# kkty/kmer-sets-compression

Measured on AMD Instinct MI355X. Metric: Mk-mers/s processed in kmerset-multiple-compress; bytes/k-mer after SPSS, higher is better.
Workload: dtype u32

## Files before the change

### kmer-sets-compression_amd/csrc/ksh_decode.hip

```cpp
#include "ksh_internal.h"
#include "ksh_kmer.h"

#include <algorithm>
#include <cstdlib>
#include <string>
#include <vector>

namespace ksh {

constexpr int kDecThreads = 1024;
constexpr int kMaxLdsBuckets = 16384;
constexpr int kSortLdsBytes = 63488;
constexpr int kMaxSubBits = 11;
constexpr int kSortThreads = 1024;

__global__ __launch_bounds__(256) void k_str_bases(const uint32_t* __restrict__ lens, int64_t n,
                                                    int k, int64_t* __restrict__ bases) {
  const int64_t i = int64_t(blockIdx.x) * blockDim.x + threadIdx.x;
  if (i < n) bases[i] = int64_t(lens[i]) + k;
}

__global__ __launch_bounds__(256) void k_mark_ends(const int64_t* __restrict__ str_start,
                                                    int64_t n_strings,
                                                    unsigned long long* __restrict__ end_bits) {
  const int64_t i = int64_t(blockIdx.x) * blockDim.x + threadIdx.x;
  if (i >= n_strings) return;
  const int64_t p = str_start[i + 1] - 1;
  atomicOr(&end_bits[p >> 6], 1ull << (p & 63));
}

__global__ __launch_bounds__(256) void k_sum_lens(const uint32_t* __restrict__ lens, int64_t n,
                                                   unsigned long long* __restrict__ out) {
  unsigned long long acc = 0;
  for (int64_t i = int64_t(blockIdx.x) * blockDim.x + threadIdx.x; i < n;
       i += int64_t(gridDim.x) * blockDim.x)
    acc += lens[i];
#pragma unroll
  for (int d = 32; d >= 1; d >>= 1) acc += __shfl_xor(acc, d, 64);
  if ((threadIdx.x & 63) == 0 && acc) atomicAdd(out, acc);
}

template <typename KeyT, bool kScatter>
__global__ __launch_bounds__(kDecThreads) void k_decode(
    const uint64_t* __restrict__ words, int64_t n_words, int64_t n_bases,
    const unsigned long long* __restrict__ end_bits, int64_t n_end_words, int k, int key_bits,
    int n_buckets, int canonical_flag, int64_t words_per_group, uint32_t* __restrict__ hist_matrix,
    const int64_t* __restrict__ offsets, KeyT* __restrict__ keys) {
  extern __shared__ uint32_t lds_hist[];
  uint32_t* my_row = hist_matrix + int64_t(blockIdx.x) * n_buckets;
  for (int b = threadIdx.x; b < n_buckets; b += kDecThreads) lds_hist[b] = kScatter ? my_row[b] : 0u;
  __syncthreads();

  const int64_t w_begin = int64_t(blockIdx.x) * words_per_group;
  const int64_t w_end = min(w_begin + words_per_group, n_words);
  const uint64_t mask = kmer_mask(k);
  const uint64_t key_mask = (uint64_t(1) << key_bits) - 1;
  const uint64_t no_end_mask = (uint64_t(1) << (k - 1)) - 1;

  for (int64_t w = w_begin + threadIdx.x; w < w_end; w += kDecThreads) {
    const uint64_t w0 = words[w];
    const uint64_t w1 = (w + 1 < n_words) ? words[w + 1] : 0;
    const int64_t p0 = w << 5;
    const int64_t ew = p0 >> 6;
    const int esh = int(p0 & 63);
    uint64_t eb = end_bits[ew] >> esh;
    if (esh && ew + 1 < n_end_words) eb |= end_bits[ew + 1] << (64 - esh);

    uint64_t fw = (k <= 32) ? (w0 >> (64 - 2 * k)) : 0;
    uint64_t rc = revcomp(fw, k);
#pragma unroll 4
    for (int j = 0; j < 32; j++) {
      const int64_t p = p0 + j;
      const bool valid = (p + k <= n_bases) && (((eb >> j) & no_end_mask) == 0);
      if (valid) {
        const uint64_t cn = (canonical_flag && rc < fw) ? rc : fw;
        const uint32_t bucket = uint32_t(cn >> key_bits);
        if (kScatter) {
          const uint32_t rel = atomicAdd(&lds_hist[bucket], 1u);
          keys[offsets[bucket] + rel] = KeyT(cn & key_mask);
        } else {
          atomicAdd(&lds_hist[bucket], 1u);
        }
      }
      const int q = j + k;
      const uint64_t nb = q < 32 ? (w0 >> (62 - 2 * q)) & 3 : (w1 >> (62 - 2 * (q - 32))) & 3;
      fw = ((fw << 2) & mask) | nb;
      rc = (rc >> 2) | ((3 - nb) << (2 * (k - 1)));
    }
  }
  if (!kScatter) {
    __syncthreads();
    for (int b = threadIdx.x; b < n_buckets; b += kDecThreads) my_row[b] = lds_hist[b];
  }
}

constexpr int kDecSgBits = 7;
constexpr int kDecL1Threads = 1024;
template <typename KeyT>
struct DecL1 {
  static constexpr int kPer = sizeof(KeyT) == 8 ? 4 : 8;
  static constexpr int kTile = kDecL1Threads * kPer;
};
constexpr int kDecL2Threads = 256;
constexpr int kDecL2Per = 8;
constexpr int kDecL2Tile = kDecL2Threads * kDecL2Per;

template <typename KeyT>
__global__ __launch_bounds__(kDecL1Threads) void k_decode_l1(
    const uint64_t* __restrict__ words, int64_t n_words, int64_t n_bases,
    const unsigned long long* __restrict__ end_bits, int64_t n_end_words, int k, int key_bits, int n_bucket_bits,
    int canonical_flag, int64_t words_per_group, const uint32_t* __restrict__ hist_matrix,
    const int64_t* __restrict__ offsets, KeyT* __restrict__ tmp_keys, uint16_t* __restrict__ tmp_b) {
  constexpr int kSg = 1 << kDecSgBits;
  constexpr int kDecL1Per = DecL1<KeyT>::kPer, kDecL1Tile = DecL1<KeyT>::kTile;
  constexpr int kParts = 32 / kDecL1Per;
  __shared__ KeyT s_key[kDecL1Tile];
  __shared__ uint16_t s_bkt[kDecL1Tile];
  __shared__ uint32_t s_cur[kSg], s_cnt[kSg], s_lbase[kSg + 1];
  const int tid = threadIdx.x;
  const int nb = 1 << n_bucket_bits, lo_bits = n_bucket_bits - kDecSgBits;
  const uint32_t* my_row = hist_matrix + int64_t(blockIdx.x) * nb;
  if (tid < kSg) {
    uint32_t at = uint32_t(offsets[int64_t(tid) << lo_bits]);
    for (int bi = 0; bi < (1 << lo_bits); bi++) at += my_row[(tid << lo_bits) + bi];
    s_cur[tid] = at;
    s_cnt[tid] = 0;
  }
  const int64_t w_begin = int64_t(blockIdx.x) * words_per_group;
  const int64_t w_end = min(w_begin + words_per_group, n_words);
  const uint64_t mask = kmer_mask(k);
  const uint64_t key_mask = (uint64_t(1) << key_bits) - 1;
  const uint64_t no_end_mask = (uint64_t(1) << (k - 1)) - 1;
  __syncthreads();
  for (int64_t w0i = w_begin; w0i < w_end; w0i += kDecL1Tile / 32) {
    const int64_t w = w0i + tid / kParts;
    const int j0 = (tid % kParts) * kDecL1Per;
    KeyT key[kDecL1Per];
    uint32_t bkt[kDecL1Per], rank[kDecL1Per];
#pragma unroll
    for (int j = 0; j < kDecL1Per; j++) bkt[j] = 0xFFFFFFFFu;
    if (w < w_end) {
      const uint64_t w0 = words[w];
      const uint64_t w1 = (w + 1 < n_words) ? words[w + 1] : 0;
      const int64_t p0 = w << 5;
      const int64_t ew = p0 >> 6;
      const int esh = int(p0 & 63);
      uint64_t eb = end_bits[ew] >> esh;
      if (esh && ew + 1 < n_end_words) eb |= end_bits[ew + 1] << (64 - esh);
      const int top = 2 * (j0 + k);
      uint64_t fw = (top <= 64 ? (w0 >> (64 - top)) : ((w0 << (top - 64)) | (w1 >> (128 - top)))) & mask;
      uint64_t rc = revcomp(fw, k);
#pragma unroll
      for (int j = 0; j < kDecL1Per; j++) {
        const int jj = j0 + j;
        const int64_t p = p0 + jj;
        const bool valid = (p + k <= n_bases) && (((eb >> jj) & no_end_mask) == 0);
        if (valid) {
          const uint64_t cn = (canonical_flag && rc < fw) ? rc : fw;
          bkt[j] = uint32_t(cn >> key_bits);
          key[j] = KeyT(cn & key_mask);
          rank[j] = atomicAdd(&s_cnt[bkt[j] >> lo_bits], 1u);
        }
        const int q = jj + k;
        const uint64_t nbase = q < 32 ? (w0 >> (62 - 2 * q)) & 3 : (w1 >> (62 - 2 * (q - 32))) & 3;
        fw = ((fw << 2) & mask) | nbase;
        rc = (rc >> 2) | ((3 - nbase) << (2 * (k - 1)));
      }
    }
    __syncthreads();
    if (tid < 64) {
      static_assert(kSg == 128, "two super-buckets per lane of one wave");
      const uint32_t c0 = s_cnt[2 * tid], c1 = s_cnt[2 * tid + 1];
      uint32_t inc = c0 + c1;
#pragma unroll
      for (int d = 1; d < 64; d <<= 1) {
        const uint32_t o = __shfl_up(inc, d, 64);
        if (tid >= d) inc += o;
      }
      s_lbase[2 * tid] = inc - c0 - c1;
      s_lbase[2 * tid + 1] = inc - c1;
      if (tid == 63) s_lbase[kSg] = inc;
    }
    __syncthreads();
#pragma unroll
    for (int j = 0; j < kDecL1Per; j++) {
      if (bkt[j] == 0xFFFFFFFFu) continue;
      const uint32_t pos = s_lbase[bkt[j] >> lo_bits] + rank[j];
      s_key[pos] = key[j];
      s_bkt[pos] = uint16_t(bkt[j]);
    }
    __syncthreads();
    const int tile_n = int(s_lbase[kSg]);
    for (int i = tid; i < tile_n; i += kDecL1Threads) {
      const uint32_t sg = uint32_t(s_bkt[i]) >> lo_bits;
      const uint32_t dst = s_cur[sg] + (uint32_t(i) - s_lbase[sg]);
      tmp_keys[dst] = s_key[i];
      tmp_b[dst] = s_bkt[i];
    }
    __syncthreads();
    if (tid < kSg) {
      s_cur[tid] += s_cnt[tid];
      s_cnt[tid] = 0;
    }
    __syncthreads();
  }
}

template <typename KeyT>
__global__ __launch_bounds__(kDecL2Threads) void k_decode_l2(int64_t n, int n_bucket_bits,
                                                             const int64_t* __restrict__ offsets,
                                                             const KeyT* __restrict__ tmp_keys,
                                                             const uint16_t* __restrict__ tmp_b,
                                                             uint32_t* __restrict__ cursor, KeyT* __restrict__ keys) {
  constexpr int kBins = 2 * kDecL2Threads;
  __shared__ KeyT s_key[kDecL2Tile];
  __shared__ uint16_t s_bin[kDecL2Tile];
  __shared__ uint32_t s_cnt[kBins], s_lbase[kBins], s_gbase[kBins];
  __shared__ uint32_t s_wave[kDecL2Threads / 64];
  __shared__ uint32_t s_first;
  const int tid = threadIdx.x;
  const int lo_bits = n_bucket_bits - kDecSgBits;
  const int64_t p0 = int64_t(blockIdx.x) * kDecL2Tile;
  const int tile_n = int(min<int64_t>(kDecL2Tile, n - p0));
  s_cnt[2 * tid] = 0;
  s_cnt[2 * tid + 1] = 0;
  if (tid == 0) s_first = (uint32_t(tmp_b[p0]) >> lo_bits) << lo_bits;
  __syncthreads();
  const uint32_t base_b = s_first;
  const uint32_t n_bins = min<uint32_t>(uint32_t(kBins), (2u << lo_bits));
  KeyT mine[kDecL2Per];
  uint32_t bin[kDecL2Per], rank[kDecL2Per];
#pragma unroll
  for (int j = 0; j < kDecL2Per; j++) {
    const int i = tid + j * kDecL2Threads;
    bin[j] = 0xFFFFFFFFu;
    if (i >= tile_n) continue;
    mine[j] = tmp_keys[p0 + i];
    const uint32_t b = tmp_b[p0 + i];
    if (b - base_b < n_bins) {
      bin[j] = b - base_b;
      rank[j] = atomicAdd(&s_cnt[bin[j]], 1u);
    } else {
      keys[uint32_t(offsets[b]) + atomicAdd(&cursor[b], 1u)] = mine[j];
    }
  }
  __syncthreads();
  {
    const uint32_t c0 = s_cnt[2 * tid], c1 = s_cnt[2 * tid + 1];
    uint32_t inc = c0 + c1;
    const int lane = tid & 63, wv = tid >> 6;
#pragma unroll
    for (int d = 1; d < 64; d <<= 1) {
      const uint32_t o = __shfl_up(inc, d, 64);
      if (lane >= d) inc += o;
    }
    if (lane == 63) s_wave[wv] = inc;
    __syncthreads();
    uint32_t before = inc - (c0 + c1);
    for (int w = 0; w < wv; w++) before += s_wave[w];
    s_lbase[2 * tid] = before;
    s_lbase[2 * tid + 1] = before + c0;
    s_gbase[2 * tid] = c0 ? uint32_t(offsets[base_b + 2 * tid]) + atomicAdd(&cursor[base_b + 2 * tid], c0) : 0u;
    s_gbase[2 * tid + 1] = c1 ? uint32_t(offsets[base_b + 2 * tid + 1]) + atomicAdd(&cursor[base_b + 2 * tid + 1], c1) : 0u;
  }
  __syncthreads();
#pragma unroll
  for (int j = 0; j < kDecL2Per; j++) {
    if (bin[j] == 0xFFFFFFFFu) continue;
    const uint32_t pos = s_lbase[bin[j]] + rank[j];
    s_key[pos] = mine[j];
    s_bin[pos] = uint16_t(bin[j]);
  }
  __syncthreads();
  const uint32_t staged = s_lbase[kBins - 1] + s_cnt[kBins - 1];
  for (uint32_t i = tid; i < staged; i += kDecL2Threads) {
    const uint32_t b = s_bin[i];
    keys[s_gbase[b] + (i - s_lbase[b])] = s_key[i];
  }
}

constexpr int kColTeams = 16;
__global__ __launch_bounds__(64 * kColTeams) void k_hist_columns(uint32_t* __restrict__ hist_matrix,
                                                                  int64_t n_groups, int n_buckets,
                                                                  int64_t* __restrict__ totals,
                                                                  unsigned long long* __restrict__ max_total) {
  __shared__ uint32_t team_total[kColTeams][64];
  const int lane = threadIdx.x & 63, team = threadIdx.x >> 6;
  const int b = blockIdx.x * 64 + lane;
  const int64_t per_team = (n_groups + kColTeams - 1) / kColTeams;
  const int64_t g0 = min(int64_t(team) * per_team, n_groups), g1 = min(g0 + per_team, n_groups);
  uint32_t run = 0;
  if (b < n_buckets)
    for (int64_t g = g0; g < g1; g++) run += hist_matrix[g * n_buckets + b];
  team_total[team][lane] = run;
  __syncthreads();
  if (b >= n_buckets) return;
  uint32_t before = 0, all = 0;
#pragma unroll
  for (int t2 = 0; t2 < kColTeams; t2++) {
    const uint32_t v = team_total[t2][lane];
    if (t2 < team) before += v;
    all += v;
  }
  run = before;
  for (int64_t g = g0; g < g1; g++) {
    uint32_t* cell = hist_matrix + g * n_buckets + b;
    const uint32_t c = *cell;
    *cell = run;
    run += c;
  }
  if (team == 0) {
    totals[b] = all;
    unsigned long long m = all;
    if (int(blockIdx.x + 1) * 64 <= n_buckets) {
#pragma unroll
      for (int d = 32; d >= 1; d >>= 1) {
        const unsigned long long o = __shfl_xor(m, d, 64);
        m = o > m ? o : m;
      }
      if (lane == 0 && max_total) atomicMax(max_total, m);
    } else if (max_total) {
      atomicMax(max_total, m);
    }
  }
}

struct SortLds {
  uint32_t sub_cnt[(1 << kMaxSubBits) + 1];
  int wave_cnt[kSortThreads / 64];
  int wave_below[kSortThreads / 64];
  int overflow;
  int kept;
};

template <typename KeyT>
__device__ void block_sort_into_lds(const KeyT* __restrict__ src, int cnt, int eff_bits,
                                    KeyT* __restrict__ lds, SortLds* __restrict__ sh) {
  int bits = 0;
  while ((4 << bits) < cnt && bits < kMaxSubBits) bits++;
  if (bits > eff_bits) bits = eff_bits;
  const int n_sub = 1 << bits;
  const int shift = eff_bits - bits;
  for (int i = threadIdx.x; i <= n_sub; i += kSortThreads) sh->sub_cnt[i] = 0;
  if (threadIdx.x == 0) sh->overflow = 0;
  constexpr int kSortRegs = 8;
  const bool in_regs = cnt <= kSortRegs * kSortThreads;
  KeyT held[kSortRegs];
  if (in_regs) {
#pragma unroll
    for (int u = 0; u < kSortRegs; u++) {
      const int i = int(threadIdx.x) + u * kSortThreads;
      if (i < cnt) held[u] = src[i];
    }
  }
  __syncthreads();
// ... 407 lines not shown
  int64_t* offw = wide ? st.coarse : d_offsets;

  const unsigned sb = unsigned((s->n_strings + 255) / 256);
  hipLaunchKernelGGL(k_str_bases, dim3(sb), dim3(256), 0, ctx->stream, s->d_lens, s->n_strings, g->k,
                     st.str_start);
  KSH_TRY(scan_exclusive_i64(ctx, st.str_start, st.str_start, s->n_strings,
                             st.str_start + s->n_strings));
  KSH_HIP(hipMemsetAsync(st.end_bits, 0, size_t(n_end_words) * 8, ctx->stream));
  hipLaunchKernelGGL(k_mark_ends, dim3(sb), dim3(256), 0, ctx->stream, st.str_start, s->n_strings,
                     st.end_bits);
  hipLaunchKernelGGL((k_decode<KeyT, false>), dim3(unsigned(groups)), dim3(kDecThreads),
                     size_t(nbw) * 4, ctx->stream, s->d_words, n_words, s->n_bases, st.end_bits,
                     n_end_words, g->k, kbw, int(nbw), canonical_flag, wpg, st.hist, nullptr,
                     static_cast<KeyT*>(nullptr));
  unsigned long long* d_max = reinterpret_cast<unsigned long long*>(st.totals + nbw + 1);
  KSH_HIP(hipMemsetAsync(d_max, 0, 8, ctx->stream));
  hipLaunchKernelGGL(k_hist_columns, dim3(unsigned((nbw + 63) / 64)), dim3(64 * kColTeams), 0, ctx->stream,
                     st.hist, groups, int(nbw), st.totals, d_max);
  KSH_TRY(scan_exclusive_i64(ctx, st.totals, offw, nbw, offw + nbw));
  if (wide)
    hipLaunchKernelGGL(k_broadcast_coarse, dim3(unsigned(nb / 256 + 1)), dim3(256), 0, ctx->stream, st.coarse,
                       g->n_bucket_bits - kCoarseBits, nb, d_offsets);
  KSH_HIP(hipGetLastError());
  KSH_HIP(hipMemcpyAsync(ctx->h_pinned, offw + nbw, 8, hipMemcpyDeviceToHost, ctx->stream));
  KSH_HIP(hipMemcpyAsync(ctx->h_pinned + 1, st.str_start + s->n_strings, 8, hipMemcpyDeviceToHost,
                         ctx->stream));
  KSH_HIP(hipMemcpyAsync(ctx->h_pinned + 2, d_max, 8, hipMemcpyDeviceToHost, ctx->stream));
  KSH_HIP(hipStreamSynchronize(ctx->stream));
  ctx->dec_max_bucket = ctx->h_pinned[2];
  if (ctx->h_pinned[1] != s->n_bases)
    return fail(KSH_INVALID_ARGUMENT, "spss: sum of string lengths (%lld) != n_bases (%lld)",
                (long long)ctx->h_pinned[1], (long long)s->n_bases);
  *n_keys = ctx->h_pinned[0];
  ctx->dec_words = n_words;
  ctx->dec_groups = groups;
  plan_done(*n_keys);
  return KSH_OK;
}

int decode_claim_plan(ksh_ctx* ctx, const char* who, const ksh_geom* g, const ksh_spss_view* s, int canonical_flag,
                      const int64_t* d_offsets) {
  if (!ctx->dec_valid)
    return fail(KSH_FAILED_PRECONDITION, "%s without a pending ksh_spss_decode_plan on this context (none made, "
                                         "replaced, failed, or already written)", who);
  const ksh_spss_view& v = ctx->dec_view;
  if (v.d_words != s->d_words || v.d_lens != s->d_lens || v.n_strings != s->n_strings || v.n_bases != s->n_bases)
    return fail(KSH_FAILED_PRECONDITION, "%s: the pending ksh_spss_decode_plan was made for another container", who);
  if (!same_geom(ctx->dec_geom, *g) || ctx->dec_canonical != (canonical_flag != 0))
    return fail(KSH_FAILED_PRECONDITION, "%s: the pending ksh_spss_decode_plan was made with another geometry "
                                         "(k, N, key bytes) or canonical flag", who);
  if (ctx->dec_offsets != d_offsets)
    return fail(KSH_FAILED_PRECONDITION, "%s: d_offsets is not the buffer the pending ksh_spss_decode_plan filled",
                who);
  return KSH_OK;
}

template <typename KeyT>
int scatter_sort(ksh_ctx* ctx, const ksh_spss_view* s, const DecodeState& st, int k, int nbits_w, int kbw,
                 int canonical_flag, const int64_t* offsets, KeyT* keys, int cutoff, bool want_below,
                 int64_t** new_off, int64_t** below) {
  const int64_t nb = int64_t(1) << nbits_w;
  int64_t n_words, n_end_words, groups, wpg;
  decode_geometry(s, &n_words, &n_end_words, &groups, &wpg);
  static const bool direct = [] {
    const char* e = getenv("KSH_DECODE_SCATTER");
    return e && std::string(e) == "direct";
  }();
  static const int64_t two_level_min = [] {
    const char* e = getenv("KSH_DECODE_L2_MIN");
    return e ? std::max<int64_t>(1024, atoll(e)) : int64_t(1) << 20;
  }();
  if (!direct && ctx->dec_kmers >= two_level_min && nbits_w > kDecSgBits && nbits_w <= 15 &&
      ctx->dec_kmers < int64_t(0xFFFFFFF0)) {
    void* tmp = nullptr;
    const size_t tk = (size_t(ctx->dec_kmers) * sizeof(KeyT) + 255) & ~size_t(255);
    KSH_TRY(pool_alloc(ctx, tk + size_t(ctx->dec_kmers) * 2 + size_t(nb) * 4 + 256, &tmp));
    KeyT* tmp_keys = static_cast<KeyT*>(tmp);
    uint16_t* tmp_b = reinterpret_cast<uint16_t*>(static_cast<char*>(tmp) + tk);
    uint32_t* cursor = reinterpret_cast<uint32_t*>(static_cast<char*>(tmp) + tk + ((size_t(ctx->dec_kmers) * 2 + 255) & ~size_t(255)));
    KSH_HIP(hipMemsetAsync(cursor, 0, size_t(nb) * 4, ctx->stream));
    hipLaunchKernelGGL((k_decode_l1<KeyT>), dim3(unsigned(groups)), dim3(kDecL1Threads), 0, ctx->stream, s->d_words,
                       n_words, s->n_bases, st.end_bits, n_end_words, k, kbw, nbits_w,
                       canonical_flag, wpg, st.hist, offsets, tmp_keys, tmp_b);
    hipLaunchKernelGGL((k_decode_l2<KeyT>), dim3(unsigned((ctx->dec_kmers + kDecL2Tile - 1) / kDecL2Tile)),
                       dim3(kDecL2Threads), 0, ctx->stream, ctx->dec_kmers, nbits_w, offsets, tmp_keys, tmp_b,
                       cursor, keys);
    pool_free(ctx, tmp);
  } else {
    hipLaunchKernelGGL((k_decode<KeyT, true>), dim3(unsigned(groups)), dim3(kDecThreads),
                       size_t(nb) * 4, ctx->stream, s->d_words, n_words, s->n_bases, st.end_bits,
                       n_end_words, k, kbw, int(nb), canonical_flag, wpg, st.hist, offsets,
                       keys);
  }
  KeyT* scratch = nullptr;
  {
    const int64_t max_bucket = ctx->dec_max_bucket;
    if (max_bucket > int64_t(kSortLdsBytes / sizeof(KeyT))) {
      void* ptr = nullptr;
      KSH_TRY(pool_alloc(ctx, size_t(ctx->dec_kmers) * sizeof(KeyT), &ptr));
      scratch = static_cast<KeyT*>(ptr);
    }
  }
  KSH_TRY(arena_layout(ctx, 1u << 16, [&](Carver& c) {
    *new_off = c.take<int64_t>(size_t(nb + 1));
    *below = c.take<int64_t>(size_t(nb + 1));
  }));
  {
    const uint32_t bit = lds_opt_in_bit<KeyT>(kLdsBucketSort);
    if (!(ctx->lds_opt_in & bit)) {
      KSH_HIP(hipFuncSetAttribute(reinterpret_cast<const void*>(k_bucket_sort<KeyT>),
                                  hipFuncAttributeMaxDynamicSharedMemorySize, kSortLdsBytes));
      ctx->lds_opt_in |= bit;
    }
  }
  hipLaunchKernelGGL((k_bucket_sort<KeyT>), dim3(unsigned(nb)), dim3(kSortThreads), kSortLdsBytes, ctx->stream,
                     offsets, keys, scratch, st.totals, kbw, cutoff, want_below ? *below : nullptr);
  if (scratch) pool_free(ctx, scratch);
  KSH_HIP(hipGetLastError());
  return KSH_OK;
}

template <typename KeyT, typename CT>
int decode_write_wide(ksh_ctx* ctx, const ksh_geom* g, const ksh_spss_view* s, int canonical_flag,
                      int64_t* d_offsets, void* d_keys, int64_t* n_keys, int cutoff, int64_t* n_below) {
  const int64_t nb = n_buckets(g), nbc = int64_t(1) << kCoarseBits;
  const int sub_bits = g->n_bucket_bits - kCoarseBits, cbits = 2 * g->k - kCoarseBits;
  int64_t n_words, n_end_words, groups, wpg;
  decode_geometry(s, &n_words, &n_end_words, &groups, &wpg);
  DecodeState st;
  KSH_TRY(decode_carve(ctx, DecodeShape{groups, nbc, n_end_words, s->n_strings, true}, &st));
  KeyT* keys = static_cast<KeyT*>(d_keys);
  constexpr bool in_place = sizeof(CT) == sizeof(KeyT);
  CT* comp = reinterpret_cast<CT*>(d_keys);
  if (!in_place) {
    void* ptr = nullptr;
    KSH_TRY(pool_alloc(ctx, size_t(ctx->dec_kmers) * sizeof(CT), &ptr));
    comp = static_cast<CT*>(ptr);
  }
  int64_t *new_off = nullptr, *below = nullptr;
  KSH_TRY(scatter_sort<CT>(ctx, s, st, g->k, kCoarseBits, cbits, canonical_flag, st.coarse, comp, cutoff,
                           n_below != nullptr, &new_off, &below));
  KSH_TRY(scan_exclusive_i64(ctx, st.totals, new_off, nbc, new_off + nbc));
  if (n_below) KSH_TRY(scan_exclusive_i64(ctx, below, below, nbc, below + nbc));
  hipLaunchKernelGGL((k_fine_offsets<CT>), dim3(unsigned(nb / 256 + 1)), dim3(256), 0, ctx->stream, st.coarse,
                     new_off, comp, sub_bits, key_bits(g), nb, d_offsets);
  KSH_HIP(hipMemcpyAsync(ctx->h_pinned, new_off + nbc, 8, hipMemcpyDeviceToHost, ctx->stream));
  if (n_below)
    KSH_HIP(hipMemcpyAsync(ctx->h_pinned + 1, below + nbc, 8, hipMemcpyDeviceToHost, ctx->stream));
  KSH_HIP(hipStreamSynchronize(ctx->stream));
  const int64_t kept = ctx->h_pinned[0];
  if (n_below) *n_below = ctx->h_pinned[1];
  const uint64_t key_mask = key_bits(g) >= 64 ? ~uint64_t(0) : (uint64_t(1) << key_bits(g)) - 1;
  void* tmp = nullptr;
  const CT* src = comp;
  if (in_place && kept != ctx->dec_kmers) {
    KSH_TRY(device_alloc(ctx, size_t(ctx->dec_kmers) * sizeof(CT), &tmp));
    KSH_HIP(hipMemcpyAsync(tmp, comp, size_t(ctx->dec_kmers) * sizeof(CT), hipMemcpyDeviceToDevice, ctx->stream));
    src = static_cast<const CT*>(tmp);
  }
  hipLaunchKernelGGL((k_narrow_buckets<CT, KeyT>), dim3(unsigned(nbc)), dim3(256), 0, ctx->stream, st.coarse,
                     new_off, src, keys, key_mask);
  KSH_HIP(hipGetLastError());
  if (!in_place) pool_free(ctx, comp);
  if (tmp) {
    KSH_HIP(hipStreamSynchronize(ctx->stream));
    KSH_HIP(hipFree(tmp));
  }
// ... 122 lines not shown
```

### kmer-sets-compression_amd/csrc/ksh_encode.hip

```cpp
#include "ksh_internal.h"
#include "ksh_dsu.h"
#include "ksh_kmer.h"

#include <algorithm>
#include <cstddef>
#include <cstdlib>
#include <string>
#ifdef KSH_EDGES_DEBUG
#include <cstdio>
#include <vector>
#endif

namespace ksh {

#ifndef KSH_RULER_SHIFT
#define KSH_RULER_SHIFT 5
#endif
constexpr int kRulerShift = KSH_RULER_SHIFT;
constexpr uint32_t kRulerEvery = 1u << kRulerShift;

constexpr uint32_t kNone = 0xFFFFFFFFu;
constexpr uint32_t kMulti = 0xFFFFFFFEu;

#ifndef KSH_JUMP_HOPS
// ... 202 lines not shown

constexpr int kColTeams = 16;
__global__ __launch_bounds__(64 * kColTeams) void k_rc_columns(uint32_t* __restrict__ hist_matrix, int64_t n_rows,
                                                                int nb, int64_t* __restrict__ totals) {
  __shared__ uint32_t team_total[kColTeams][64];
  const int lane = threadIdx.x & 63, team = threadIdx.x >> 6;
  const int b = blockIdx.x * 64 + lane;
  const int64_t per_team = (n_rows + kColTeams - 1) / kColTeams;
  const int64_t g0 = min(int64_t(team) * per_team, n_rows), g1 = min(g0 + per_team, n_rows);
  uint32_t run = 0;
  if (b < nb)
    for (int64_t g = g0; g < g1; g++) run += hist_matrix[g * nb + b];
  team_total[team][lane] = run;
  __syncthreads();
  if (b >= nb) return;
  uint32_t before = 0, all = 0;
#pragma unroll
  for (int t2 = 0; t2 < kColTeams; t2++) {
    const uint32_t v = team_total[t2][lane];
    if (t2 < team) before += v;
    all += v;
  }
  run = before;
  for (int64_t g = g0; g < g1; g++) {
    uint32_t* cell = hist_matrix + g * nb + b;
    const uint32_t c = *cell;
    *cell = run;
    run += c;
  }
  if (team == 0) totals[b] = all;
}

template <typename KeyT>
__global__ __launch_bounds__(1024) void k_rc_scatter(DevSet<KeyT> set, int nbits, int round_bits, int round,
                                                      int64_t per_row,
                                                      const uint32_t* __restrict__ hist_matrix,
                                                      const int64_t* __restrict__ goff,
                                                      RcRecord<KeyT>* __restrict__ rec) {
  extern __shared__ uint32_t lds_hist[];
  const int nb = 1 << nbits;
  const uint32_t* my_row = hist_matrix + int64_t(blockIdx.x) * nb;
  for (int b = threadIdx.x; b < nb; b += blockDim.x) lds_hist[b] = uint32_t(goff[b]) + my_row[b];
  const int64_t t_begin = int64_t(blockIdx.x) * per_row;
  const int64_t t_end = min(t_begin + per_row, set.n);
  __syncthreads();
  if (t_begin >= t_end) return;
  const int64_t b_first = set.bucket_of(t_begin), b_last = set.bucket_of(t_end - 1);
  const int k = set.k, low_bits = 2 * set.k - 2 - nbits;
  const uint64_t low_mask = (uint64_t(1) << low_bits) - 1;
  for (int64_t t = t_begin + threadIdx.x; t < t_end; t += blockDim.x) {
    const uint64_t key = uint64_t(set.keys[t]);
    const uint32_t grp = uint32_t(revcomp(key, k) >> low_bits) & uint32_t(nb - 1);
    if (int(grp >> (nbits - round_bits)) != round) continue;
    int64_t lo = b_first, hi = b_last;
    while (lo < hi) {
      const int64_t mid = (lo + hi + 1) >> 1;
      if (set.off[mid] <= t) lo = mid; else hi = mid - 1;
    }
    const uint64_t rx = revcomp((uint64_t(lo) << set.key_bits) | key, k);
    const uint32_t dst = atomicAdd(&lds_hist[grp], 1u);
    RcRecord<KeyT> r;
    r.key = KeyT(((rx >> (2 * k - 2)) << low_bits) | (rx & low_mask));
    r.t = uint32_t(t);
    rec[dst] = r;
  }
}

constexpr int kSgBits = 7;
constexpr int kL1Threads = 1024;
constexpr int kL2Threads = 256;
constexpr int kL2Per = 8;
constexpr int kL2Tile = kL2Threads * kL2Per;

template <typename KeyT, int kPer>
__global__ __launch_bounds__(kL1Threads) void k_rc_scatter_l1(DevSet<KeyT> set, int nbits, int64_t per_row,
                                                               const uint32_t* __restrict__ hist_matrix,
                                                               const int64_t* __restrict__ goff,
                                                               RcRecord<KeyT>* __restrict__ tmp_rec,
                                                               uint16_t* __restrict__ tmp_g) {
  constexpr int kTile = kL1Threads * kPer;
  constexpr int kSg = 1 << kSgBits;
  __shared__ RcRecord<KeyT> s_rec[kTile];
  __shared__ uint16_t s_g[kTile];
  __shared__ uint32_t s_cur[kSg], s_cnt[kSg], s_lbase[kSg + 1];
  constexpr int kOffCap = 1024;
  __shared__ int64_t s_off[kOffCap];
  const int tid = threadIdx.x;
  const int nb = 1 << nbits, lo_bits = nbits - kSgBits;
  const uint32_t* my_row = hist_matrix + int64_t(blockIdx.x) * nb;
  if (tid < kSg) {
    uint32_t at = uint32_t(goff[int64_t(tid) << lo_bits]);
    for (int gi = 0; gi < (1 << lo_bits); gi++) at += my_row[(tid << lo_bits) + gi];
    s_cur[tid] = at;
    s_cnt[tid] = 0;
  }
  const int64_t t_begin = int64_t(blockIdx.x) * per_row;
  const int64_t t_end = min(t_begin + per_row, set.n);
  __syncthreads();
  if (t_begin >= t_end) return;
  const int64_t b_first = set.bucket_of(t_begin), b_last = set.bucket_of(t_end - 1);
  const int k = set.k, low_bits = 2 * set.k - 2 - nbits;
  const uint64_t low_mask = (uint64_t(1) << low_bits) - 1;
  const int n_span = int(min<int64_t>(b_last - b_first + 1, kOffCap + 1));
  const bool off_staged = n_span <= kOffCap;
  if (off_staged)
    for (int j = tid; j < n_span; j += kL1Threads) s_off[j] = set.off[b_first + j];
  __syncthreads();
  for (int64_t t0 = t_begin; t0 < t_end; t0 += kTile) {
    const int tile_n = int(min<int64_t>(kTile, t_end - t0));
    RcRecord<KeyT> mine[kPer];
    uint32_t grp[kPer], rank[kPer];
#pragma unroll
    for (int j = 0; j < kPer; j++) {
      const int64_t t = t0 + tid + j * kL1Threads;
      grp[j] = 0xFFFFFFFFu;
      if (t >= t_end) continue;
      const uint64_t key = uint64_t(set.keys[t]);
      int64_t lo = b_first, hi = b_last;
      if (off_staged) {
        int l2 = 0, h2 = n_span - 1;
        while (l2 < h2) {
          const int mid = (l2 + h2 + 1) >> 1;
          if (s_off[mid] <= t) l2 = mid; else h2 = mid - 1;
        }
        lo = b_first + l2;
      } else {
        while (lo < hi) {
          const int64_t mid = (lo + hi + 1) >> 1;
          if (set.off[mid] <= t) lo = mid; else hi = mid - 1;
        }
      }
      const uint64_t rx = revcomp((uint64_t(lo) << set.key_bits) | key, k);
      grp[j] = uint32_t(rx >> low_bits) & uint32_t(nb - 1);
      mine[j].key = KeyT(((rx >> (2 * k - 2)) << low_bits) | (rx & low_mask));
      mine[j].t = uint32_t(t);
      rank[j] = atomicAdd(&s_cnt[grp[j] >> lo_bits], 1u);
    }
    __syncthreads();
    if (tid < 64) {
      static_assert(kSg == 128, "two super-groups per lane of one wave");
      const uint32_t c0 = s_cnt[2 * tid], c1 = s_cnt[2 * tid + 1];
      uint32_t inc = c0 + c1;
#pragma unroll
      for (int d = 1; d < 64; d <<= 1) {
        const uint32_t o = __shfl_up(inc, d, 64);
        if (tid >= d) inc += o;
      }
      s_lbase[2 * tid] = inc - c0 - c1;
      s_lbase[2 * tid + 1] = inc - c1;
    }
    __syncthreads();
#pragma unroll
    for (int j = 0; j < kPer; j++) {
      if (grp[j] == 0xFFFFFFFFu) continue;
      const uint32_t pos = s_lbase[grp[j] >> lo_bits] + rank[j];
      s_rec[pos] = mine[j];
      s_g[pos] = uint16_t(grp[j]);
    }
    __syncthreads();
    for (int i = tid; i < tile_n; i += kL1Threads) {
      const uint32_t sg = uint32_t(s_g[i]) >> lo_bits;
      const uint32_t dst = s_cur[sg] + (uint32_t(i) - s_lbase[sg]);
      tmp_rec[dst] = s_rec[i];
      tmp_g[dst] = s_g[i];
    }
    __syncthreads();
    if (tid < kSg) {
      s_cur[tid] += s_cnt[tid];
      s_cnt[tid] = 0;
    }
    __syncthreads();
  }
}

template <typename KeyT>
__global__ __launch_bounds__(kL2Threads) void k_rc_scatter_l2(int64_t n, int nbits, const int64_t* __restrict__ goff,
                                                               const RcRecord<KeyT>* __restrict__ tmp_rec,
                                                               const uint16_t* __restrict__ tmp_g,
                                                               uint32_t* __restrict__ cursor,
                                                               RcRecord<KeyT>* __restrict__ rec) {
  constexpr int kBins = 512;
  __shared__ RcRecord<KeyT> s_rec[kL2Tile];
  __shared__ uint16_t s_bin[kL2Tile];
  __shared__ uint32_t s_cnt[kBins], s_lbase[kBins], s_gbase[kBins];
  __shared__ uint32_t s_first;
  const int tid = threadIdx.x;
  const int lo_bits = nbits - kSgBits;
  const int64_t p0 = int64_t(blockIdx.x) * kL2Tile;
  const int tile_n = int(min<int64_t>(kL2Tile, n - p0));
  for (int b = tid; b < kBins; b += kL2Threads) s_cnt[b] = 0;
  if (tid == 0) s_first = (uint32_t(tmp_g[p0]) >> lo_bits) << lo_bits;
  __syncthreads();
  const uint32_t base_g = s_first;
  const uint32_t n_bins = min<uint32_t>(uint32_t(kBins), (2u << lo_bits));
  RcRecord<KeyT> mine[kL2Per];
  uint32_t bin[kL2Per], rank[kL2Per];
#pragma unroll
  for (int j = 0; j < kL2Per; j++) {
    const int i = tid + j * kL2Threads;
    bin[j] = 0xFFFFFFFFu;
    if (i >= tile_n) continue;
    mine[j] = tmp_rec[p0 + i];
    const uint32_t g = tmp_g[p0 + i];
    if (g - base_g < n_bins) {
      bin[j] = g - base_g;
      rank[j] = atomicAdd(&s_cnt[bin[j]], 1u);
    } else {
      rec[uint32_t(goff[g]) + atomicAdd(&cursor[g], 1u)] = mine[j];
    }
  }
  __syncthreads();
  {
    static_assert(kBins == 2 * kL2Threads, "two bins per thread");
    __shared__ uint32_t s_wave[kL2Threads / 64];
    const uint32_t c0 = s_cnt[2 * tid], c1 = s_cnt[2 * tid + 1];
    uint32_t inc = c0 + c1;
    const int lane = tid & 63, wv = tid >> 6;
#pragma unroll
    for (int d = 1; d < 64; d <<= 1) {
      const uint32_t o = __shfl_up(inc, d, 64);
      if (lane >= d) inc += o;
    }
    if (lane == 63) s_wave[wv] = inc;
    __syncthreads();
    uint32_t before = inc - (c0 + c1);
    for (int w = 0; w < wv; w++) before += s_wave[w];
    s_lbase[2 * tid] = before;
    s_lbase[2 * tid + 1] = before + c0;
    s_gbase[2 * tid] = c0 ? uint32_t(goff[base_g + 2 * tid]) + atomicAdd(&cursor[base_g + 2 * tid], c0) : 0u;
    s_gbase[2 * tid + 1] = c1 ? uint32_t(goff[base_g + 2 * tid + 1]) + atomicAdd(&cursor[base_g + 2 * tid + 1], c1) : 0u;
  }
  __syncthreads();
#pragma unroll
  for (int j = 0; j < kL2Per; j++) {
    if (bin[j] == 0xFFFFFFFFu) continue;
    const uint32_t pos = s_lbase[bin[j]] + rank[j];
    s_rec[pos] = mine[j];
    s_bin[pos] = uint16_t(bin[j]);
  }
  __syncthreads();
  uint32_t staged = 0;
  for (int b = 0; b < kBins; b++) staged += s_cnt[b];
  for (uint32_t i = tid; i < staged; i += kL2Threads) {
    const uint32_t b = s_bin[i];
    rec[s_gbase[b] + (i - s_lbase[b])] = s_rec[i];
  }
}

template <typename KeyT>
__device__ int64_t lower_bound_kmer(const DevSet<KeyT>& set, uint64_t value) {
  const int64_t b = int64_t(value >> set.key_bits);
  if (b >= set.n_buckets) return set.n;
  const KeyT key = KeyT(value & set.key_mask());
  int64_t lo, hi;
  set.probe_range(b, key, &lo, &hi);
  while (lo < hi) {
    const int64_t mid = (lo + hi) >> 1;
    if (set.keys[mid] < key) lo = mid + 1; else hi = mid;
  }
  return lo;
}

__device__ __forceinline__ void mark_hit(uint32_t* slot, uint32_t v) {
  if (atomicCAS(slot, kNone, v) != kNone) *reinterpret_cast<volatile uint32_t*>(slot) = kMulti;
}

constexpr int kRcSegs = 16;

template <typename KeyT>
__global__ __launch_bounds__(256) void k_rc_bounds(DevSet<KeyT> set, int nbits, int64_t* __restrict__ pb,
                                                    int64_t* __restrict__ pb0) {
  const int64_t i = int64_t(blockIdx.x) * blockDim.x + threadIdx.x;
  const int64_t n_pb = int64_t(2 * kRcSegs) << nbits;
  if (i < n_pb) {
    const uint64_t grp = uint64_t(i) >> 5, seg = (uint64_t(i) >> 1) & 15, which = uint64_t(i) & 1;
    const uint64_t prefix = (seg << nbits) | grp;
    pb[i] = lower_bound_kmer(set, (prefix + which) << (2 * set.k - 4 - nbits));
  } else if (pb0 && i - n_pb < (int64_t(2) << nbits)) {
    const uint64_t j = uint64_t(i - n_pb);
    pb0[j] = lower_bound_kmer(set, ((j >> 1) + (j & 1)) << (2 * set.k - nbits));
  }
}
struct RcBatch {
  int64_t seg_lo[kRcSegs], seg_hi[kRcSegs];
  int64_t win_lo[kRcSegs];
  int win_len[kRcSegs];
  int win_off[kRcSegs];
  int idx_off[kRcSegs];
  int idx_shift[kRcSegs];
  unsigned long long packed[kRcSegs];
  int used;
  int next_seg;
  int64_t next_pos;
};

template <typename KeyT, int kRcThreads>
__global__ __launch_bounds__(kRcThreads, (kRcThreads >= 512 ? 8 : (kRcThreads >= 128 ? kRcThreads / 128 : 1))) void k_adj_rc(
    DevSet<KeyT> set, int gbits, const int64_t* __restrict__ goff, const RcRecord<KeyT>* __restrict__ rec,
    const int64_t* __restrict__ pb, const int64_t* __restrict__ pb0, int cap, uint32_t* __restrict__ rc0,
    uint32_t* __restrict__ rc1, int* __restrict__ batched, int pass1_cap, int* __restrict__ taken) {
  extern __shared__ __attribute__((aligned(16))) unsigned char lds_raw[];
  KeyT* skeys = reinterpret_cast<KeyT*>(lds_raw);
  uint32_t* slots = reinterpret_cast<uint32_t*>(lds_raw + size_t(cap) * sizeof(KeyT));
  uint16_t* sidx = reinterpret_cast<uint16_t*>(lds_raw + size_t(cap) * (sizeof(KeyT) + 4));
  __shared__ RcBatch bt;
  __shared__ int64_t prev_bounds[2 * kRcSegs];
  static_assert(kRcThreads % kRcSegs == 0, "pass 1 deals the ranges out to sixteen teams");
  constexpr int kTeam = kRcThreads / kRcSegs;
  const int tid = threadIdx.x, lane = tid % kTeam, wave = tid / kTeam;
  const int64_t grp = blockIdx.x;
  const int k = set.k, low_bits = 2 * set.k - 2 - gbits;
  const int extra = gbits - int(2 * set.k - set.key_bits);
  const uint64_t low_mask = (uint64_t(1) << low_bits) - 1;
  const uint64_t kmask = kmer_mask(k);
  const int64_t r0 = goff[grp], r1 = goff[grp + 1];
  if (r1 - r0 <= int64_t(pass1_cap)) return;
  if (pass1_cap >= 0 && threadIdx.x == 0) *taken = 1;
  const int64_t p0_lo = pb0 ? pb0[2 * grp] : set.off[grp], p0_hi = pb0 ? pb0[2 * grp + 1] : set.off[grp + 1];
  const uint64_t gkey_top = extra > 0 ? (uint64_t(grp) & ((uint64_t(1) << extra) - 1)) << (set.key_bits - extra) : 0;
  KSH_PMARK_WAVE(2);
  if (tid < 2 * kRcSegs) prev_bounds[tid] = pb[2 * kRcSegs * grp + tid];
  KSH_PMARK(1, 0);
  for (int pass = 0; pass < 2; pass++) {
    const int n_seg = pass == 0 ? 1 : kRcSegs;
    const int seg_bits = (pass == 0 ? set.key_bits : set.key_bits - 4) - extra;
// ... 3403 lines not shown
```

Measured before the change: 28600.

## Prefetch next tile inputs and overlap global atomics in decode/encode scatter kernels

The decode L1 kernel now loads the next tile's words and end-bit words into registers while the current tile is processed. The encode L1 kernel prefetches keys one tile ahead, tracks the bucket index incrementally instead of running a fresh binary search per element, and folds the cursor update into the scan so two barriers per tile go away. The L2 scatter kernels issue all global loads before the shared-memory barrier, start the global cursor atomics before the prefix scan, and the decode L2 tile doubles for 32-bit keys. The aim is to hide memory latency and cut barriers, at the cost of more registers and LDS, which may lower occupancy.

```diff
diff --git a/kmer-sets-compression_amd/csrc/ksh_decode.hip b/kmer-sets-compression_amd/csrc/ksh_decode.hip
--- a/kmer-sets-compression_amd/csrc/ksh_decode.hip
+++ b/kmer-sets-compression_amd/csrc/ksh_decode.hip
@@ -102,8 +102,11 @@
   static constexpr int kTile = kDecL1Threads * kPer;
 };
 constexpr int kDecL2Threads = 256;
-constexpr int kDecL2Per = 8;
-constexpr int kDecL2Tile = kDecL2Threads * kDecL2Per;
+template <typename KeyT>
+struct DecL2 {
+  static constexpr int kPer = sizeof(KeyT) == 8 ? 8 : 16;
+  static constexpr int kTile = kDecL2Threads * kPer;
+};
 
 template <typename KeyT>
 __global__ __launch_bounds__(kDecL1Threads) void k_decode_l1(
@@ -132,6 +135,16 @@
   const uint64_t key_mask = (uint64_t(1) << key_bits) - 1;
   const uint64_t no_end_mask = (uint64_t(1) << (k - 1)) - 1;
   __syncthreads();
+  uint64_t a_w0 = 0, a_w1 = 0, a_e0 = 0, a_e1 = 0;
+  const auto ask = [&](int64_t w) {
+    if (w >= w_end) return;
+    a_w0 = words[w];
+    a_w1 = (w + 1 < n_words) ? words[w + 1] : 0;
+    const int64_t ew = w >> 1;
+    a_e0 = end_bits[ew];
+    a_e1 = ((w & 1) && ew + 1 < n_end_words) ? end_bits[ew + 1] : 0;
+  };
+  ask(w_begin + tid / kParts);
   for (int64_t w0i = w_begin; w0i < w_end; w0i += kDecL1Tile / 32) {
     const int64_t w = w0i + tid / kParts;
     const int j0 = (tid % kParts) * kDecL1Per;
@@ -139,14 +152,13 @@
     uint32_t bkt[kDecL1Per], rank[kDecL1Per];
 #pragma unroll
     for (int j = 0; j < kDecL1Per; j++) bkt[j] = 0xFFFFFFFFu;
+    const uint64_t w0 = a_w0, w1 = a_w1, e0 = a_e0, e1 = a_e1;
+    ask(w + kDecL1Tile / 32);
     if (w < w_end) {
-      const uint64_t w0 = words[w];
-      const uint64_t w1 = (w + 1 < n_words) ? words[w + 1] : 0;
       const int64_t p0 = w << 5;
-      const int64_t ew = p0 >> 6;
       const int esh = int(p0 & 63);
-      uint64_t eb = end_bits[ew] >> esh;
-      if (esh && ew + 1 < n_end_words) eb |= end_bits[ew + 1] << (64 - esh);
+      uint64_t eb = e0 >> esh;
+      if (esh) eb |= e1 << (64 - esh);
       const int top = 2 * (j0 + k);
       uint64_t fw = (top <= 64 ? (w0 >> (64 - top)) : ((w0 << (top - 64)) | (w1 >> (128 - top)))) & mask;
       uint64_t rc = revcomp(fw, k);
@@ -213,30 +225,35 @@
                                                              const uint16_t* __restrict__ tmp_b,
                                                              uint32_t* __restrict__ cursor, KeyT* __restrict__ keys) {
   constexpr int kBins = 2 * kDecL2Threads;
+  constexpr int kDecL2Per = DecL2<KeyT>::kPer, kDecL2Tile = DecL2<KeyT>::kTile;
   __shared__ KeyT s_key[kDecL2Tile];
   __shared__ uint16_t s_bin[kDecL2Tile];
   __shared__ uint32_t s_cnt[kBins], s_lbase[kBins], s_gbase[kBins];
   __shared__ uint32_t s_wave[kDecL2Threads / 64];
-  __shared__ uint32_t s_first;
   const int tid = threadIdx.x;
   const int lo_bits = n_bucket_bits - kDecSgBits;
   const int64_t p0 = int64_t(blockIdx.x) * kDecL2Tile;
   const int tile_n = int(min<int64_t>(kDecL2Tile, n - p0));
   s_cnt[2 * tid] = 0;
   s_cnt[2 * tid + 1] = 0;
-  if (tid == 0) s_first = (uint32_t(tmp_b[p0]) >> lo_bits) << lo_bits;
-  __syncthreads();
-  const uint32_t base_b = s_first;
+  const uint32_t base_b = (uint32_t(tmp_b[p0]) >> lo_bits) << lo_bits;
   const uint32_t n_bins = min<uint32_t>(uint32_t(kBins), (2u << lo_bits));
   KeyT mine[kDecL2Per];
-  uint32_t bin[kDecL2Per], rank[kDecL2Per];
+  uint32_t bid[kDecL2Per], bin[kDecL2Per], rank[kDecL2Per];
+#pragma unroll
+  for (int j = 0; j < kDecL2Per; j++) {
+    const int i = tid + j * kDecL2Threads;
+    if (i >= tile_n) continue;
+    mine[j] = tmp_keys[p0 + i];
+    bid[j] = tmp_b[p0 + i];
+  }
+  __syncthreads();
 #pragma unroll
   for (int j = 0; j < kDecL2Per; j++) {
     const int i = tid + j * kDecL2Threads;
     bin[j] = 0xFFFFFFFFu;
     if (i >= tile_n) continue;
-    mine[j] = tmp_keys[p0 + i];
-    const uint32_t b = tmp_b[p0 + i];
+    const uint32_t b = bid[j];
     if (b - base_b < n_bins) {
       bin[j] = b - base_b;
       rank[j] = atomicAdd(&s_cnt[bin[j]], 1u);
@@ -245,8 +262,11 @@
     }
   }
   __syncthreads();
+  uint32_t g0 = 0, g1 = 0;
   {
     const uint32_t c0 = s_cnt[2 * tid], c1 = s_cnt[2 * tid + 1];
+    if (c0) g0 = uint32_t(offsets[base_b + 2 * tid]) + atomicAdd(&cursor[base_b + 2 * tid], c0);
+    if (c1) g1 = uint32_t(offsets[base_b + 2 * tid + 1]) + atomicAdd(&cursor[base_b + 2 * tid + 1], c1);
     uint32_t inc = c0 + c1;
     const int lane = tid & 63, wv = tid >> 6;
 #pragma unroll
@@ -260,8 +280,6 @@
     for (int w = 0; w < wv; w++) before += s_wave[w];
     s_lbase[2 * tid] = before;
     s_lbase[2 * tid + 1] = before + c0;
-    s_gbase[2 * tid] = c0 ? uint32_t(offsets[base_b + 2 * tid]) + atomicAdd(&cursor[base_b + 2 * tid], c0) : 0u;
-    s_gbase[2 * tid + 1] = c1 ? uint32_t(offsets[base_b + 2 * tid + 1]) + atomicAdd(&cursor[base_b + 2 * tid + 1], c1) : 0u;
   }
   __syncthreads();
 #pragma unroll
@@ -271,6 +289,8 @@
     s_key[pos] = mine[j];
     s_bin[pos] = uint16_t(bin[j]);
   }
+  s_gbase[2 * tid] = g0;
+  s_gbase[2 * tid + 1] = g1;
   __syncthreads();
   const uint32_t staged = s_lbase[kBins - 1] + s_cnt[kBins - 1];
   for (uint32_t i = tid; i < staged; i += kDecL2Threads) {
@@ -844,7 +864,7 @@
     hipLaunchKernelGGL((k_decode_l1<KeyT>), dim3(unsigned(groups)), dim3(kDecL1Threads), 0, ctx->stream, s->d_words,
                        n_words, s->n_bases, st.end_bits, n_end_words, k, kbw, nbits_w,
                        canonical_flag, wpg, st.hist, offsets, tmp_keys, tmp_b);
-    hipLaunchKernelGGL((k_decode_l2<KeyT>), dim3(unsigned((ctx->dec_kmers + kDecL2Tile - 1) / kDecL2Tile)),
+    hipLaunchKernelGGL((k_decode_l2<KeyT>), dim3(unsigned((ctx->dec_kmers + DecL2<KeyT>::kTile - 1) / DecL2<KeyT>::kTile)),
                        dim3(kDecL2Threads), 0, ctx->stream, ctx->dec_kmers, nbits_w, offsets, tmp_keys, tmp_b,
                        cursor, keys);
     pool_free(ctx, tmp);
diff --git a/kmer-sets-compression_amd/csrc/ksh_encode.hip b/kmer-sets-compression_amd/csrc/ksh_encode.hip
--- a/kmer-sets-compression_amd/csrc/ksh_encode.hip
+++ b/kmer-sets-compression_amd/csrc/ksh_encode.hip
@@ -308,7 +308,7 @@
   constexpr int kSg = 1 << kSgBits;
   __shared__ RcRecord<KeyT> s_rec[kTile];
   __shared__ uint16_t s_g[kTile];
-  __shared__ uint32_t s_cur[kSg], s_cnt[kSg], s_lbase[kSg + 1];
+  __shared__ uint32_t s_cur[kSg], s_cnt[kSg], s_lbase[kSg + 1], s_dst[kSg];
   constexpr int kOffCap = 1024;
   __shared__ int64_t s_off[kOffCap];
   const int tid = threadIdx.x;
@@ -332,24 +332,52 @@
   if (off_staged)
     for (int j = tid; j < n_span; j += kL1Threads) s_off[j] = set.off[b_first + j];
   __syncthreads();
+  int at_b = 0;
+  if (off_staged) {
+    const int64_t t = min(t_begin + tid, t_end - 1);
+    int h2 = n_span - 1;
+    while (at_b < h2) {
+      const int mid = (at_b + h2 + 1) >> 1;
+      if (s_off[mid] <= t) at_b = mid; else h2 = mid - 1;
+    }
+  }
+  KeyT ahead[kPer];
+#pragma unroll
+  for (int j = 0; j < kPer; j++) {
+    const int64_t t = t_begin + tid + j * kL1Threads;
+    ahead[j] = t < t_end ? set.keys[t] : KeyT(0);
+  }
   for (int64_t t0 = t_begin; t0 < t_end; t0 += kTile) {
     const int tile_n = int(min<int64_t>(kTile, t_end - t0));
     RcRecord<KeyT> mine[kPer];
     uint32_t grp[kPer], rank[kPer];
+    KeyT now[kPer];
+#pragma unroll
+    for (int j = 0; j < kPer; j++) {
+      now[j] = ahead[j];
+      const int64_t t = t0 + kTile + tid + j * kL1Threads;
+      ahead[j] = t < t_end ? set.keys[t] : KeyT(0);
+    }
 #pragma unroll
     for (int j = 0; j < kPer; j++) {
       const int64_t t = t0 + tid + j * kL1Threads;
       grp[j] = 0xFFFFFFFFu;
       if (t >= t_end) continue;
-      const uint64_t key = uint64_t(set.keys[t]);
+      const uint64_t key = uint64_t(now[j]);
       int64_t lo = b_first, hi = b_last;
       if (off_staged) {
-        int l2 = 0, h2 = n_span - 1;
-        while (l2 < h2) {
-          const int mid = (l2 + h2 + 1) >> 1;
-          if (s_off[mid] <= t) l2 = mid; else h2 = mid - 1;
+        if (at_b + 1 < n_span && s_off[at_b + 1] <= t) {
+          at_b++;
+          if (at_b + 1 < n_span && s_off[at_b + 1] <= t) {
+            int h2 = n_span - 1;
+            at_b++;
+            while (at_b < h2) {
+              const int mid = (at_b + h2 + 1) >> 1;
+              if (s_off[mid] <= t) at_b = mid; else h2 = mid - 1;
+            }
+          }
         }
-        lo = b_first + l2;
+        lo = b_first + at_b;
       } else {
         while (lo < hi) {
           const int64_t mid = (lo + hi + 1) >> 1;
@@ -366,14 +394,22 @@
     if (tid < 64) {
       static_assert(kSg == 128, "two super-groups per lane of one wave");
       const uint32_t c0 = s_cnt[2 * tid], c1 = s_cnt[2 * tid + 1];
+      s_cnt[2 * tid] = 0;
+      s_cnt[2 * tid + 1] = 0;
       uint32_t inc = c0 + c1;
 #pragma unroll
       for (int d = 1; d < 64; d <<= 1) {
         const uint32_t o = __shfl_up(inc, d, 64);
         if (tid >= d) inc += o;
       }
-      s_lbase[2 * tid] = inc - c0 - c1;
-      s_lbase[2 * tid + 1] = inc - c1;
+      const uint32_t l0 = inc - c0 - c1, l1 = inc - c1;
+      s_lbase[2 * tid] = l0;
+      s_lbase[2 * tid + 1] = l1;
+      const uint32_t cur0 = s_cur[2 * tid], cur1 = s_cur[2 * tid + 1];
+      s_dst[2 * tid] = cur0 - l0;
+      s_dst[2 * tid + 1] = cur1 - l1;
+      s_cur[2 * tid] = cur0 + c0;
+      s_cur[2 * tid + 1] = cur1 + c1;
     }
     __syncthreads();
 #pragma unroll
@@ -385,17 +421,11 @@
     }
     __syncthreads();
     for (int i = tid; i < tile_n; i += kL1Threads) {
-      const uint32_t sg = uint32_t(s_g[i]) >> lo_bits;
-      const uint32_t dst = s_cur[sg] + (uint32_t(i) - s_lbase[sg]);
+      const uint32_t g = s_g[i];
+      const uint32_t dst = s_dst[g >> lo_bits] + uint32_t(i);
       tmp_rec[dst] = s_rec[i];
-      tmp_g[dst] = s_g[i];
-    }
-    __syncthreads();
-    if (tid < kSg) {
-      s_cur[tid] += s_cnt[tid];
-      s_cnt[tid] = 0;
-    }
-    __syncthreads();
+      tmp_g[dst] = uint16_t(g);
+    }
   }
 }
 
@@ -409,25 +439,29 @@
   __shared__ RcRecord<KeyT> s_rec[kL2Tile];
   __shared__ uint16_t s_bin[kL2Tile];
   __shared__ uint32_t s_cnt[kBins], s_lbase[kBins], s_gbase[kBins];
-  __shared__ uint32_t s_first;
   const int tid = threadIdx.x;
   const int lo_bits = nbits - kSgBits;
   const int64_t p0 = int64_t(blockIdx.x) * kL2Tile;
   const int tile_n = int(min<int64_t>(kL2Tile, n - p0));
   for (int b = tid; b < kBins; b += kL2Threads) s_cnt[b] = 0;
-  if (tid == 0) s_first = (uint32_t(tmp_g[p0]) >> lo_bits) << lo_bits;
-  __syncthreads();
-  const uint32_t base_g = s_first;
+  const uint32_t base_g = (uint32_t(tmp_g[p0]) >> lo_bits) << lo_bits;
   const uint32_t n_bins = min<uint32_t>(uint32_t(kBins), (2u << lo_bits));
   RcRecord<KeyT> mine[kL2Per];
-  uint32_t bin[kL2Per], rank[kL2Per];
+  uint32_t gid[kL2Per], bin[kL2Per], rank[kL2Per];
+#pragma unroll
+  for (int j = 0; j < kL2Per; j++) {
+    const int i = tid + j * kL2Threads;
+    if (i >= tile_n) continue;
+    mine[j] = tmp_rec[p0 + i];
+    gid[j] = tmp_g[p0 + i];
+  }
+  __syncthreads();
 #pragma unroll
   for (int j = 0; j < kL2Per; j++) {
     const int i = tid + j * kL2Threads;
     bin[j] = 0xFFFFFFFFu;
     if (i >= tile_n) continue;
-    mine[j] = tmp_rec[p0 + i];
-    const uint32_t g = tmp_g[p0 + i];
+    const uint32_t g = gid[j];
     if (g - base_g < n_bins) {
       bin[j] = g - base_g;
       rank[j] = atomicAdd(&s_cnt[bin[j]], 1u);
@@ -436,10 +470,13 @@
     }
   }
   __syncthreads();
+  uint32_t g0 = 0, g1 = 0;
   {
     static_assert(kBins == 2 * kL2Threads, "two bins per thread");
     __shared__ uint32_t s_wave[kL2Threads / 64];
     const uint32_t c0 = s_cnt[2 * tid], c1 = s_cnt[2 * tid + 1];
+    if (c0) g0 = uint32_t(goff[base_g + 2 * tid]) + atomicAdd(&cursor[base_g + 2 * tid], c0);
+    if (c1) g1 = uint32_t(goff[base_g + 2 * tid + 1]) + atomicAdd(&cursor[base_g + 2 * tid + 1], c1);
     uint32_t inc = c0 + c1;
     const int lane = tid & 63, wv = tid >> 6;
 #pragma unroll
@@ -453,8 +490,6 @@
     for (int w = 0; w < wv; w++) before += s_wave[w];
     s_lbase[2 * tid] = before;
     s_lbase[2 * tid + 1] = before + c0;
-    s_gbase[2 * tid] = c0 ? uint32_t(goff[base_g + 2 * tid]) + atomicAdd(&cursor[base_g + 2 * tid], c0) : 0u;
-    s_gbase[2 * tid + 1] = c1 ? uint32_t(goff[base_g + 2 * tid + 1]) + atomicAdd(&cursor[base_g + 2 * tid + 1], c1) : 0u;
   }
   __syncthreads();
 #pragma unroll
@@ -464,9 +499,10 @@
     s_rec[pos] = mine[j];
     s_bin[pos] = uint16_t(bin[j]);
   }
+  s_gbase[2 * tid] = g0;
+  s_gbase[2 * tid + 1] = g1;
   __syncthreads();
-  uint32_t staged = 0;
-  for (int b = 0; b < kBins; b++) staged += s_cnt[b];
+  const uint32_t staged = s_lbase[kBins - 1] + s_cnt[kBins - 1];
   for (uint32_t i = tid; i < staged; i += kL2Threads) {
     const uint32_t b = s_bin[i];
     rec[s_gbase[b] + (i - s_lbase[b])] = s_rec[i];
```

Result: no change. 28990, median of 6 (+1.4%).
